# 011235813/discrete_mean_field_game

Measured on AMD Instinct MI355X. Metric: env-steps/sec for batched d-bin population rollouts, higher is better.
Workload: dtype f32 (f64 accumulate); 1 GPU; actor_critic.train(update_every="rollout") of the drop-in class (mfg_ac2.train call surface; device-side start draw every episode, one update per 15-step rollout): d=21 topics, T=15, global batch 65536 = 65536 trajectories per GPU x 1; d=21, T=15, batch_per_gpu=65536, global_batch=65536, rng=philox4x32-10, parallelism=trajectory-sharded x1, 1 all-reduce/update

## Files before the change

### discrete_mean_field_game_amd/csrc/mfg_grad.h

```cpp
#pragma once
#include <hip/hip_runtime.h>
#include <stdint.h>

#include "mfg_core.h"

using namespace mfg;

constexpr int MFG_GRAD_SMALL_MAX_D = 28;
constexpr int GR_OUT_PER_THREAD = 4;
constexpr int GR_OUT_PER_BLOCK = GR_OUT_PER_THREAD * BLOCK;

struct GradArgs {
  const float* pi;
  int64_t stride_b;
  const double* delta;
  const double* g;
  const float* reward;
  int64_t N;
  int T, d, chunk;
  int64_t nsb;
  double* partial;
  int add_reward;
  unsigned* counter;
  double* G;
  int accumulate, apply;
  double lr_c, lr_a;
  double *w, *theta, *reward_acc;
};

__device__ __forceinline__ void grad_partial_body(const GradArgs& a) {
  extern __shared__ __attribute__((aligned(16))) unsigned char smem_raw[];
  const int d = a.d, Q = d * (d + 1) / 2, F = Q + d + 1, FO = F + 3;
  double* dl = reinterpret_cast<double*>(smem_raw);
  float* sp = reinterpret_cast<float*>(dl + 3 * a.chunk);
  const int tid = threadIdx.x;
  int oi[GR_OUT_PER_THREAD], oj[GR_OUT_PER_THREAD], kind[GR_OUT_PER_THREAD];
  double acc[GR_OUT_PER_THREAD];
#pragma unroll
  for (int u = 0; u < GR_OUT_PER_THREAD; ++u) {
    const int k = blockIdx.y * GR_OUT_PER_BLOCK + u * BLOCK + tid;
    acc[u] = 0.0;
    oi[u] = oj[u] = 0;
    if (k < Q) {
      int i = (int)(((2.0 * d + 1.0) - sqrt((2.0 * d + 1.0) * (2.0 * d + 1.0) - 8.0 * (double)k)) * 0.5);
      while (i > 0 && feat_idx(i, i, d) > k) --i;
      while (i + 1 < d && feat_idx(i + 1, i + 1, d) <= k) ++i;
      oi[u] = i;
      oj[u] = i + (k - feat_idx(i, i, d));
      kind[u] = 0;
    } else if (k < Q + d) {
      oi[u] = k - Q;
      kind[u] = 1;
    } else if (k < FO) {
      kind[u] = 2 + (k - (Q + d));
    } else {
      kind[u] = -1;
    }
  }
  for (int64_t n0 = (int64_t)blockIdx.x * a.chunk; n0 < a.N; n0 += a.nsb * a.chunk) {
    const int cn = (int)((a.N - n0) < a.chunk ? (a.N - n0) : a.chunk);
    __syncthreads();
    for (int k = tid; k < cn * d; k += BLOCK) {
      const int q = k / d, c = k - q * d;
      const int64_t n = n0 + q;
      const int64_t b = n / a.T;
      const int s = (int)(n - b * a.T);
      sp[k] = a.pi[b * a.stride_b + (int64_t)s * d + c];
    }
    for (int q = tid; q < cn; q += BLOCK) {
      const double de = a.delta[n0 + q];
      dl[3 * q] = de;
      dl[3 * q + 1] = a.g ? de * a.g[n0 + q] : 0.0;
      dl[3 * q + 2] = a.reward ? (double)a.reward[n0 + q] : 0.0;
    }
    __syncthreads();
#pragma unroll
    for (int u = 0; u < GR_OUT_PER_THREAD; ++u) {
      double s_ = acc[u];
      if (kind[u] == 0) {
        for (int q = 0; q < cn; ++q) s_ = fma(dl[3 * q] * (double)sp[q * d + oi[u]], (double)sp[q * d + oj[u]], s_);
      } else if (kind[u] == 1) {
        for (int q = 0; q < cn; ++q) s_ = fma(dl[3 * q], (double)sp[q * d + oi[u]], s_);
      } else if (kind[u] == 2) {
        for (int q = 0; q < cn; ++q) s_ += dl[3 * q];
      } else if (kind[u] == 3) {
        for (int q = 0; q < cn; ++q) s_ += dl[3 * q + 1];
      } else if (kind[u] == 4) {
        for (int q = 0; q < cn; ++q) s_ += dl[3 * q + 2];
      } else if (kind[u] == 5) {
        s_ += (double)cn;
      }
      acc[u] = s_;
    }
  }
#pragma unroll
  for (int u = 0; u < GR_OUT_PER_THREAD; ++u) {
    const int k = blockIdx.y * GR_OUT_PER_BLOCK + u * BLOCK + tid;
    if (kind[u] >= 0) a.partial[(int64_t)blockIdx.x * FO + k] = acc[u];
  }
}

constexpr int GS_CH = 64;
#ifndef MFG_GS_BPC
#define MFG_GS_BPC 2
#endif

template <int D>
struct GradChunk {
  static constexpr int NL = D ? D : MFG_GRAD_SMALL_MAX_D;
  float pi[NL];
  double de, dg;
  float rr;
};

constexpr int MFG_GRAD_LONG_T = 1 << 22;
__device__ __forceinline__ int grad_boundaries_wide(int sj, int T, float invT) {
  return T >= GS_CH ? (int)(sj >= T) : (int)(((float)sj + 0.5f) * invT);
}
template <int D, bool WIDE>
__device__ __forceinline__ void grad_chunk_load(GradChunk<D>& c, const GradArgs& a, const double* gp, const float* rp, int d,
                                                int64_t n0, int64_t b0, int s0, int lane, float invT, float inv_d) {
  const int last = (int)((a.N - 1 - n0) < (GS_CH - 1) ? (a.N - 1 - n0) : (GS_CH - 1));
  {
    const int64_t n = n0 + (lane < last ? lane : last);
    c.de = a.delta[n];
    c.dg = gp[n];
    c.rr = rp[n];
  }
  if constexpr (!WIDE) {
    const float* cb = a.pi + b0 * a.stride_b + (int64_t)s0 * d;
    const int extra = (int)(a.stride_b - (int64_t)a.T * d);
#pragma unroll
    for (int k = 0; k < GradChunk<D>::NL; ++k) {
      if (!D && k * WAVE >= GS_CH * d) {
        c.pi[k] = 0.0f;
        continue;
      }
      int e = k * WAVE + lane;
      int j = (int)(((float)e + 0.5f) * inv_d);
      if (j > last) { j = last; e = last * d; }
      const int q = (int)(((float)(s0 + j) + 0.5f) * invT);
      c.pi[k] = cb[(unsigned)(e + __mul24(q, extra))];
    }
  } else {
#pragma unroll
    for (int k = 0; k < GradChunk<D>::NL; ++k) {
      if (!D && k * WAVE >= GS_CH * d) {
        c.pi[k] = 0.0f;
        continue;
      }
      const int e = k * WAVE + lane;
      int j = (int)(((float)e + 0.5f) * inv_d);
      int col = e - j * d;
      if (j > last) { j = last; col = 0; }
      const int sj = s0 + j;
      const int q = grad_boundaries_wide(sj, a.T, invT);
      const int64_t off = (b0 + q) * a.stride_b + ((int64_t)(sj - q * a.T) * d + col);
      c.pi[k] = a.pi[off];
    }
  }
}

template <int D, bool WIDE>
__device__ __forceinline__ void grad_mfma_small_body(const GradArgs& a) {
  const int d = D ? D : a.d;
  const int Q = d * (d + 1) / 2, F = Q + d + 1, FO = F + 3;
  constexpr int DMAX = D ? D : MFG_GRAD_SMALL_MAX_D;
  constexpr int PI_FL = GS_CH * DMAX + 16;
  constexpr int W_BYTES = ((PI_FL * 4 + 15) / 16) * 16 + GS_CH * 3 * 8;
  constexpr int RED_BYTES = WAVES * 3 * 4 * WAVE * 8;
  __shared__ __attribute__((aligned(16))) unsigned char smem[(WAVES * W_BYTES > RED_BYTES) ? WAVES * W_BYTES : RED_BYTES];
  const int tid = threadIdx.x, lane = tid & (WAVE - 1), wv = __builtin_amdgcn_readfirstlane(tid / WAVE);
  float* lpi = reinterpret_cast<float*>(smem + (size_t)wv * W_BYTES);
  double* lsc = reinterpret_cast<double*>(smem + (size_t)wv * W_BYTES + ((PI_FL * 4 + 15) / 16) * 16);
  const int li = lane & 15, lk = lane >> 4;
  auto consts = [&](int idx, float& a_d, double& a_1, float& b_1, double& b_g, double& b_r) {
    a_d = idx == d ? 1.0f : 0.0f;
    a_1 = idx == d + 1 ? 1.0 : 0.0;
    b_1 = (idx == d || idx == d + 3) ? 1.0f : 0.0f;
    b_g = idx == d + 1 ? 1.0 : 0.0;
    b_r = idx == d + 2 ? 1.0 : 0.0;
  };
  float ad_lo, b1_lo, ad_hi, b1_hi;
  double a1_lo, a1_hi, bg_lo, br_lo, bg_hi, br_hi;
  consts(li, ad_lo, a1_lo, b1_lo, bg_lo, br_lo);
  consts(16 + li, ad_hi, a1_hi, b1_hi, bg_hi, br_hi);
  const bool pi_lo = li < d, pi_hi = 16 + li < d;
  const int ilo = pi_lo ? li : 0, ihi = pi_hi ? 16 + li : 0;
  const bool has_g = a.g != nullptr, has_r = a.reward != nullptr;
  const double* gp = has_g ? a.g : a.delta;
  const float* rp = has_r ? a.reward : a.pi;
  v4d_t c00 = (v4d_t)(0.0), c01 = (v4d_t)(0.0), c11 = (v4d_t)(0.0);
  const float invT = 1.0f / (float)a.T, inv_d = 1.0f / (float)d;
  const int64_t NC = (a.N + GS_CH - 1) / GS_CH;
  const int64_t W = (int64_t)gridDim.x * WAVES;
  const int64_t gw = (int64_t)blockIdx.x * WAVES + wv;
  GradChunk<D> nx;
  if (gw < NC) grad_chunk_load<D, WIDE>(nx, a, gp, rp, d, gw * GS_CH, (gw * GS_CH) / a.T, (int)((gw * GS_CH) % a.T), lane, invT, inv_d);
  for (int64_t ch = gw; ch < NC; ch += W) {
    const int64_t n0 = ch * GS_CH;
    __builtin_amdgcn_s_waitcnt(0xc07f);
    __builtin_amdgcn_wave_barrier();
#pragma unroll
    for (int k = 0; k < GradChunk<D>::NL; ++k)
      if (D || k * WAVE < GS_CH * d) lpi[k * WAVE + lane] = nx.pi[k];
    {
      const bool ok = n0 + lane < a.N;
      const double rr = (ok && has_r) ? (double)nx.rr : 0.0;
      double de = ok ? nx.de : 0.0;
      if (a.add_reward) {
        de += rr;
        if (ok) const_cast<double*>(a.delta)[n0 + lane] = de;
      }
      lsc[3 * lane] = de;
      lsc[3 * lane + 1] = (ok && has_g) ? nx.dg : 0.0;
      lsc[3 * lane + 2] = rr;
    }
    const int nvalid = (int)((a.N - n0) < GS_CH ? (a.N - n0) : GS_CH);
    if (ch + W < NC) {
      const int64_t n1 = (ch + W) * GS_CH;
      grad_chunk_load<D, WIDE>(nx, a, gp, rp, d, n1, n1 / a.T, (int)(n1 % a.T), lane, invT, inv_d);
    }
    __builtin_amdgcn_s_waitcnt(0xc07f);
    __builtin_amdgcn_wave_barrier();
#pragma unroll 4
    for (int ks = 0; ks < GS_CH / 4; ++ks) {
      const int j = 4 * ks + lk;
      const float plo = lpi[j * d + ilo], phi = lpi[j * d + ihi];
      const double de = lsc[3 * j], dg = lsc[3 * j + 1];
      const double rr = lsc[3 * j + 2];
      const double one = j < nvalid ? 1.0 : 0.0;
      double A_lo, B_lo;
      if constexpr (D >= 16) {
        B_lo = (double)plo;
        A_lo = de * B_lo;
      } else {
        A_lo = fma(de, (double)(pi_lo ? plo : ad_lo), a1_lo * one);
        B_lo = fma(bg_lo, dg, fma(br_lo, rr, (double)(pi_lo ? plo : b1_lo)));
      }
      const double A_hi = fma(de, (double)(pi_hi ? phi : ad_hi), a1_hi * one);
      const double B_hi = fma(bg_hi, dg, fma(br_hi, rr, (double)(pi_hi ? phi : b1_hi)));
      c00 = __builtin_amdgcn_mfma_f64_16x16x4f64(A_lo, B_lo, c00, 0, 0, 0);
      c01 = __builtin_amdgcn_mfma_f64_16x16x4f64(A_lo, B_hi, c01, 0, 0, 0);
      c11 = __builtin_amdgcn_mfma_f64_16x16x4f64(A_hi, B_hi, c11, 0, 0, 0);
    }
  }
  __syncthreads();
  double (*red)[3][4][WAVE] = reinterpret_cast<double (*)[3][4][WAVE]>(smem);
#pragma unroll
  for (int v = 0; v < 4; ++v) {
    red[wv][0][v][lane] = c00[v];
    red[wv][1][v][lane] = c01[v];
    red[wv][2][v][lane] = c11[v];
  }
  __syncthreads();
  double* out = a.partial + (int64_t)blockIdx.x * FO;
  for (int e = tid; e < 3 * 4 * WAVE; e += BLOCK) {
    const int t = e / (4 * WAVE), v = (e / WAVE) & 3, l = e & (WAVE - 1);
    const int gi = (t == 2 ? 16 : 0) + 4 * v + (l >> 4), gj = (t == 0 ? 0 : 16) + (l & 15);
    int k = -1;
    if (gj < d) {
      if (gi <= gj) k = feat_idx(gi, gj, d);
    } else if (gj == d) {
      if (gi <= d) k = Q + gi;
    } else if (gj == d + 1) {
      if (gi == d) k = F;
    } else if (gj == d + 2) {
      if (gi == d + 1) k = F + 1;
    } else if (gj == d + 3) {
      if (gi == d + 1) k = F + 2;
    }
    if (k >= 0) {
      double tsum = red[0][t][v][l];
#pragma unroll
      for (int q = 1; q < WAVES; ++q) tsum += red[q][t][v][l];
      out[k] = tsum;
    }
  }
  if (!a.counter) return;
  __shared__ int s_last;
  __threadfence();
  __syncthreads();
  if (tid == 0) s_last = (atomicAdd(a.counter, 1u) == gridDim.x - 1) ? 1 : 0;
  __syncthreads();
  if (!s_last) return;
  __threadfence();
  double* fin = &red[0][0][0][0];
  const int nrows = (int)gridDim.x;
  for (int k = tid; k < FO; k += BLOCK) {
    double s0 = 0.0, s1 = 0.0, s2 = 0.0, s3 = 0.0;
    const double* col = a.partial + k;
    int r = 0;
    for (; r + 7 < nrows; r += 8) {
      const double v0 = col[(int64_t)r * FO], v1 = col[(int64_t)(r + 1) * FO], v2 = col[(int64_t)(r + 2) * FO],
                   v3 = col[(int64_t)(r + 3) * FO], v4 = col[(int64_t)(r + 4) * FO], v5 = col[(int64_t)(r + 5) * FO],
                   v6 = col[(int64_t)(r + 6) * FO], v7 = col[(int64_t)(r + 7) * FO];
      s0 += v0;
      s1 += v1;
      s2 += v2;
      s3 += v3;
      s0 += v4;
      s1 += v5;
      s2 += v6;
      s3 += v7;
    }
    for (; r < nrows; ++r) s0 += col[(int64_t)r * FO];
    const double tot = (s0 + s1) + (s2 + s3);
    const double gk = a.accumulate ? a.G[k] + tot : tot;
    a.G[k] = gk;
    fin[k] = gk;
  }
  __syncthreads();
  if (a.apply) {
    const double count = fin[F + 2];
    if (count > 0.0) {
      const double inv = 1.0 / count;
      for (int k = tid; k < F; k += BLOCK) a.w[k] = updated_param(a.w[k], a.lr_c, fin[k], inv);
      if (tid == 0) {
        if (a.reward_acc) *a.reward_acc += fin[F + 1] * inv;
        *a.theta = updated_param(*a.theta, a.lr_a, fin[F], inv);
      }
    }
  }
  if (tid == 0) *a.counter = 0u;
}
template <int D, bool WIDE = false>
__global__ __launch_bounds__(BLOCK) void k_grad_mfma_small(GradArgs a) { grad_mfma_small_body<D, WIDE>(a); }

constexpr int GM_KC = 32;
#ifndef MFG_GM_TPW
#define MFG_GM_TPW 8
#endif
constexpr int GM_TPW = MFG_GM_TPW;

template <int NPF>
__device__ __forceinline__ void grad_mfma_body(const GradArgs& a, int tpw) {
  extern __shared__ __attribute__((aligned(16))) unsigned char smem_raw[];
  const int d = a.d, nt = d >> 4, pitch = d + 16;
  const int Q = d * (d + 1) / 2, F = Q + d + 1, FO = F + 3;
  double* dl = reinterpret_cast<double*>(smem_raw);
  double* red = dl + GM_KC;
  float* sp = reinterpret_cast<float*>(red + 4 * BLOCK);
  const int tid = threadIdx.x, lane = tid & (WAVE - 1), wv = tid / WAVE;
  const int ntiles = nt * (nt + 1) / 2;
  const int t0 = ((int)blockIdx.y * WAVES + wv) * tpw;
  int nmine = ntiles - t0;
  nmine = nmine < 0 ? 0 : (nmine > tpw ? tpw : nmine);
  int tr[GM_TPW], tc[GM_TPW];
#pragma unroll
  for (int i = 0; i < GM_TPW; ++i) {
    int t = t0 + i, r = 0;
    if (i < nmine) {
      while (t >= nt - r) {
        t -= nt - r;
        ++r;
      }
    } else {
      t = 0;
    }
    tr[i] = r;
    tc[i] = r + t;
  }
  v4d_t acc[GM_TPW];
#pragma unroll
  for (int i = 0; i < GM_TPW; ++i) acc[i] = (v4d_t)(0.0);
  const bool side = blockIdx.y == 0;
  double lin[4] = {0.0, 0.0, 0.0, 0.0}, s_d = 0.0, s_dg = 0.0, s_r = 0.0, s_n = 0.0;
  const int li = lane & 15, lk = lane >> 4;
  const double invT = 1.0 / (double)a.T;
  const int dq = d >> 2, rpp = BLOCK / (dq > 0 ? dq : 1);
  const int q0 = tid / dq, c4 = tid - q0 * dq;
  float4 pf[NPF > 0 ? NPF : 1];
  double pf_de = 0.0, pf_dg = 0.0, pf_rr = 0.0;
  bool pf_on = false;
#define MFG_GM_FETCH(n0_)                                                                              \
  {                                                                                                    \
    const int cn_ = (int)((a.N - (n0_)) < GM_KC ? (a.N - (n0_)) : GM_KC);                              \
    _Pragma("unroll") for (int u = 0; u < NPF; ++u) {                                                  \
      const int q = q0 + u * rpp;                                                                      \
      pf[u] = make_float4(0.f, 0.f, 0.f, 0.f);                                                         \
      if (q < cn_) {                                                                                   \
        const int64_t n = (n0_) + q;                                                                   \
        const int64_t b = (int64_t)(((double)n + 0.5) * invT);                                         \
        pf[u] = *reinterpret_cast<const float4*>(a.pi + b * a.stride_b + (n - b * a.T) * d + 4 * c4);  \
      }                                                                                                \
    }                                                                                                  \
    pf_de = 0.0; pf_dg = 0.0; pf_rr = 0.0; pf_on = false;                                              \
    if (tid < cn_) {                                                                                   \
      const int64_t n = (n0_) + tid;                                                                   \
      pf_de = a.delta[n];                                                                              \
      pf_rr = a.reward ? (double)a.reward[n] : 0.0;                                                    \
      if (a.g) pf_dg = a.g[n];                                                                         \
      pf_on = true;                                                                                    \
    }                                                                                                  \
  }
  if (NPF > 0 && (int64_t)blockIdx.x * GM_KC < a.N) MFG_GM_FETCH((int64_t)blockIdx.x * GM_KC)
  for (int64_t n0 = (int64_t)blockIdx.x * GM_KC; n0 < a.N; n0 += (int64_t)gridDim.x * GM_KC) {
    const int cn = (int)((a.N - n0) < GM_KC ? (a.N - n0) : GM_KC);
    __syncthreads();
    if (NPF > 0) {
#pragma unroll
      for (int u = 0; u < NPF; ++u) *reinterpret_cast<float4*>(sp + (q0 + u * rpp) * pitch + 4 * c4) = pf[u];
      if (tid < GM_KC) {
        if (side && pf_on) {
          s_d += pf_de;
          if (a.g) s_dg = fma(pf_de, pf_dg, s_dg);
          s_r += pf_rr;
          s_n += 1.0;
        }
        dl[tid] = pf_de;
      }
      __syncthreads();
      const int64_t nn = n0 + (int64_t)gridDim.x * GM_KC;
      if (nn < a.N) MFG_GM_FETCH(nn)
    } else {
    if (a.chunk) {
      for (int q = q0; q < GM_KC; q += rpp) {
        float4 v = make_float4(0.f, 0.f, 0.f, 0.f);
        if (q < cn) {
          const int64_t n = n0 + q;
          const int64_t b = (int64_t)(((double)n + 0.5) * invT);
          v = *reinterpret_cast<const float4*>(a.pi + b * a.stride_b + (n - b * a.T) * d + 4 * c4);
        }
        *reinterpret_cast<float4*>(sp + q * pitch + 4 * c4) = v;
      }
    } else {
      for (int k = tid; k < GM_KC * d; k += BLOCK) {
        const int q = k / d, c = k - q * d;
        float v = 0.0f;
        if (q < cn) {
          const int64_t n = n0 + q;
          const int64_t b = (int64_t)(((double)n + 0.5) * invT);
          v = a.pi[b * a.stride_b + (n - b * a.T) * d + c];
        }
        sp[q * pitch + c] = v;
      }
    }
    if (tid < GM_KC) {
      double de = 0.0;
      if (tid < cn) {
        const int64_t n = n0 + tid;
        de = a.delta[n];
        const double rr = a.reward ? (double)a.reward[n] : 0.0;
        if (side) {
          s_d += de;
          if (a.g) s_dg = fma(de, a.g[n], s_dg);
          s_r += rr;
          s_n += 1.0;
        }
      }
      dl[tid] = de;
    }
    __syncthreads();
    }
#pragma unroll
    for (int ks = 0; ks < GM_KC / 4; ++ks) {
      const int k = ks * 4 + lk;
      const double dk = dl[k];
      const float* row = sp + k * pitch + li;
#pragma unroll
      for (int i = 0; i < GM_TPW; ++i) {
        if (i < nmine) {
          const double av = dk * (double)row[tr[i] << 4];
          const double bv = (double)row[tc[i] << 4];
          acc[i] = __builtin_amdgcn_mfma_f64_16x16x4f64(av, bv, acc[i], 0, 0, 0);
        }
      }
    }
    if (side) {
#pragma unroll
      for (int u = 0; u < 4; ++u) {
        const int c = tid + u * BLOCK;
        if (c < d) {
          double t = lin[u];
          for (int q = 0; q < GM_KC; ++q) t = fma(dl[q], (double)sp[q * pitch + c], t);
          lin[u] = t;
        }
      }
    }
  }
#undef MFG_GM_FETCH
  double* out = a.partial + (int64_t)blockIdx.x * FO;
#pragma unroll
  for (int i = 0; i < GM_TPW; ++i) {
    if (i < nmine) {
#pragma unroll
      for (int v = 0; v < 4; ++v) {
        const int gi = (tr[i] << 4) + 4 * v + lk, gj = (tc[i] << 4) + li;
        if (gi <= gj) out[feat_idx(gi, gj, d)] = acc[i][v];
      }
    }
  }
  if (side) {
#pragma unroll
    for (int u = 0; u < 4; ++u) {
      const int c = tid + u * BLOCK;
      if (c < d) out[Q + c] = lin[u];
    }
    __syncthreads();
    red[tid] = s_d;
    red[BLOCK + tid] = s_dg;
    red[2 * BLOCK + tid] = s_r;
    red[3 * BLOCK + tid] = s_n;
    __syncthreads();
    if (tid < 4) {
      double t = 0.0;
      for (int q = 0; q < GM_KC; ++q) t += red[tid * BLOCK + q];
      out[Q + d + tid] = t;
    }
  }
}
template <int NPF>
__global__ __launch_bounds__(BLOCK) void k_grad_mfma(GradArgs a, int tpw) { grad_mfma_body<NPF>(a, tpw); }

constexpr int RP_SLICES = 64, RP_OUT = 16;
struct ReduceApply {
  double lr_c, lr_a, count;
  double *w, *theta, *reward_acc;
  int on;
};
__device__ __forceinline__ void reduce_partials_body(const double* __restrict__ partial, int64_t nsb, int64_t FO, int accumulate,
                                                     double* __restrict__ G, const ReduceApply& ap) {
  __shared__ double red[RP_SLICES][RP_OUT + 1];
  const int lo = threadIdx.x & (RP_OUT - 1), sl = threadIdx.x / RP_OUT;
  const int64_t k = (int64_t)blockIdx.x * RP_OUT + lo;
  double old_val = 0.0, old_G = 0.0;
  if (sl == 0 && k < FO) {
    const int64_t F = FO - 3;
    if (accumulate) old_G = G[k];
    if (ap.on) {
      if (k < F) old_val = ap.w[k];
      else if (k == F) old_val = *ap.theta;
      else if (k == F + 1 && ap.reward_acc) old_val = *ap.reward_acc;
    }
  }
  double s = 0.0;
  if (k < FO) {
    double s0 = 0.0, s1 = 0.0, s2 = 0.0, s3 = 0.0;
    int64_t p = sl;
    for (; p + 7 * RP_SLICES < nsb; p += 8 * RP_SLICES) {
      const double v0 = partial[p * FO + k], v1 = partial[(p + RP_SLICES) * FO + k], v2 = partial[(p + 2 * RP_SLICES) * FO + k],
                   v3 = partial[(p + 3 * RP_SLICES) * FO + k], v4 = partial[(p + 4 * RP_SLICES) * FO + k],
                   v5 = partial[(p + 5 * RP_SLICES) * FO + k], v6 = partial[(p + 6 * RP_SLICES) * FO + k],
                   v7 = partial[(p + 7 * RP_SLICES) * FO + k];
      s0 += v0;
      s1 += v1;
      s2 += v2;
      s3 += v3;
      s0 += v4;
      s1 += v5;
      s2 += v6;
      s3 += v7;
    }
    double t[7];
#pragma unroll
    for (int u = 0; u < 7; ++u) t[u] = (p + u * RP_SLICES < nsb) ? partial[(p + u * RP_SLICES) * FO + k] : 0.0;
    s0 += t[0];
    s1 += t[1];
    s2 += t[2];
    s3 += t[3];
    s0 += t[4];
    s1 += t[5];
    s2 += t[6];
    s = (s0 + s1) + (s2 + s3);
  }
  red[sl][lo] = s;
  __syncthreads();
  if (sl == 0 && k < FO) {
    double t0 = 0.0, t1 = 0.0, t2 = 0.0, t3 = 0.0;
#pragma unroll
    for (int q = 0; q < RP_SLICES; q += 4) {
      t0 += red[q][lo];
      t1 += red[q + 1][lo];
      t2 += red[q + 2][lo];
      t3 += red[q + 3][lo];
    }
    const double tot = (t0 + t1) + (t2 + t3);
    const double gk = accumulate ? old_G + tot : tot;
    G[k] = gk;
    if (ap.on) {
      const int64_t F = FO - 3;
      const double inv = 1.0 / ap.count;
      if (k < F) ap.w[k] = updated_param(old_val, ap.lr_c, gk, inv);
      else if (k == F) *ap.theta = updated_param(old_val, ap.lr_a, gk, inv);
      else if (k == F + 1 && ap.reward_acc) *ap.reward_acc = old_val + gk * inv;
    }
  }
}
```

### discrete_mean_field_game_amd/csrc/mfg_population.hip

```cpp
#include "mfg_core.h"
#include "mfg_grad.h"
#include "mfg_population.h"
#include "mfg_population_core.h"

namespace mfg {

int launch_core_pop(const CoreArgs& a, const PopArgs& p, bool fast, int num_cus, hipStream_t st) {
  return p.state ? launch_core_pop_ctl(a, p, fast, num_cus, st) : launch_core_pop_forms<false>(a, p, fast, num_cus, st);
}

__global__ void k_draw_start_pop(const float* __restrict__ mat, int64_t num_start, int64_t B, int d, uint32_t step,
                                 uint64_t traj_offset, float* __restrict__ out, PopArgs p) {
  const int k = blockIdx.y;
  draw_start_body(mat, num_start, B, d, p.seed[k], step, traj_offset, nullptr, out + p.s_state * k);
}
__global__ void k_draw_start_pop_ctl(const float* __restrict__ mat, int64_t num_start, int64_t B, int d, uint32_t step,
                                     uint64_t traj_offset, float* __restrict__ out, PopArgs p) {
  const int k = blockIdx.y;
  if (pop_retired(p, k)) return;
  draw_start_body(mat, num_start, B, d, p.seed[k], step, traj_offset, nullptr, out + p.s_state * k);
}

void launch_draw_start_pop(int grid, const float* mat, int64_t num_start, int64_t B, int d, uint32_t step, uint64_t traj_offset,
                           float* out, const PopArgs& p, hipStream_t st) {
  hipLaunchKernelGGL(p.state ? k_draw_start_pop_ctl : k_draw_start_pop, dim3((unsigned)grid, (unsigned)p.K), dim3(256), 0, st, mat,
                     num_start, B, d, step, traj_offset, out, p);
}

__device__ __forceinline__ void pop_rebase_grad(GradArgs& a, const PopArgs& p, int k) {
  a.pi += p.s_gpi * k;
  a.delta += p.s_n * k;
  a.g += p.s_n * k;
  a.reward = pop_at(a.reward, p.s_n, k);
  a.partial = pop_bytes(a.partial, p.s_ws, k);
  a.counter = pop_bytes(a.counter, p.s_ws, k);
  a.G = pop_at(a.G, p.F + 3, k);
  a.w = pop_at(a.w, p.F, k);
  a.theta = pop_at(a.theta, 1, k);
  a.reward_acc = pop_at(a.reward_acc, p.s_acc, k);
  a.lr_c = p.lr_c[k] * p.sc;
  a.lr_a = p.lr_a[k] * p.sa;
}

template <int D>
__global__ __launch_bounds__(BLOCK) void k_grad_mfma_small_pop(GradArgs a, PopArgs p) {
  GradArgs b = a;
  pop_rebase_grad(b, p, blockIdx.y);
  grad_mfma_small_body<D, false>(b);
}
template <int D>
__global__ __launch_bounds__(BLOCK) void k_grad_mfma_small_pop_ctl(GradArgs a, PopArgs p) {
  if (pop_retired(p, blockIdx.y)) return;
  GradArgs b = a;
  pop_rebase_grad(b, p, blockIdx.y);
  grad_mfma_small_body<D, false>(b);
}

__global__ __launch_bounds__(BLOCK) void k_grad_partial_pop(GradArgs a, PopArgs p) {
  GradArgs b = a;
  pop_rebase_grad(b, p, blockIdx.z);
  grad_partial_body(b);
}
__global__ __launch_bounds__(BLOCK) void k_grad_partial_pop_ctl(GradArgs a, PopArgs p) {
  if (pop_retired(p, blockIdx.z)) return;
  GradArgs b = a;
  pop_rebase_grad(b, p, blockIdx.z);
  grad_partial_body(b);
}

template <int NPF>
__global__ __launch_bounds__(BLOCK) void k_grad_mfma_pop(GradArgs a, int tpw, PopArgs p) {
  GradArgs b = a;
  pop_rebase_grad(b, p, blockIdx.z);
  grad_mfma_body<NPF>(b, tpw);
}
template <int NPF>
__global__ __launch_bounds__(BLOCK) void k_grad_mfma_pop_ctl(GradArgs a, int tpw, PopArgs p) {
  if (pop_retired(p, blockIdx.z)) return;
  GradArgs b = a;
  pop_rebase_grad(b, p, blockIdx.z);
  grad_mfma_body<NPF>(b, tpw);
}

#define MFG_REDUCE_PARTIALS_POP()                                                                                        \
  ReduceApply q = ap;                                                                                                    \
  if (q.on) {                                                                                                            \
    q.w = pop_at(ap.w, p.F, k);                                                                                          \
    q.theta = pop_at(ap.theta, 1, k);                                                                                    \
    q.reward_acc = pop_at(ap.reward_acc, p.s_acc, k);                                                                    \
    q.lr_c = p.lr_c[k] * p.sc;                                                                                           \
    q.lr_a = p.lr_a[k] * p.sa;                                                                                           \
  }                                                                                                                      \
                         \
  reduce_partials_body(reinterpret_cast<const double*>(reinterpret_cast<const char*>(partial) + p.s_ws * k), nsb, FO, 0, \
                       G + FO * k, q)
__global__ __launch_bounds__(RP_SLICES* RP_OUT) void k_reduce_partials_pop(const double* __restrict__ partial, int64_t nsb,
                                                                          int64_t FO, double* __restrict__ G, ReduceApply ap,
                                                                          PopArgs p) {
  const int k = blockIdx.y;
  MFG_REDUCE_PARTIALS_POP();
}
__global__ __launch_bounds__(RP_SLICES* RP_OUT) void k_reduce_partials_pop_ctl(const double* __restrict__ partial, int64_t nsb,
                                                                              int64_t FO, double* __restrict__ G, ReduceApply ap,
                                                                              PopArgs p) {
  const int k = blockIdx.y;
  if (pop_retired(p, k)) return;
  MFG_REDUCE_PARTIALS_POP();
}
#undef MFG_REDUCE_PARTIALS_POP

void launch_grad_mfma_small_pop(int D, unsigned blocks, const GradArgs& a, const PopArgs& p, hipStream_t st) {
  const dim3 grid(blocks, (unsigned)p.K);
  auto* k = D == 21   ? (p.state ? k_grad_mfma_small_pop_ctl<21> : k_grad_mfma_small_pop<21>)
            : D == 15 ? (p.state ? k_grad_mfma_small_pop_ctl<15> : k_grad_mfma_small_pop<15>)
                      : (p.state ? k_grad_mfma_small_pop_ctl<0> : k_grad_mfma_small_pop<0>);
  hipLaunchKernelGGL(k, grid, dim3(BLOCK), 0, st, a, p);
}

void launch_grad_partial_pop(unsigned nsb, unsigned nob, size_t lds, const GradArgs& a, const PopArgs& p, hipStream_t st) {
  hipLaunchKernelGGL(p.state ? k_grad_partial_pop_ctl : k_grad_partial_pop, dim3(nsb, nob, (unsigned)p.K), dim3(BLOCK), lds, st, a,
                     p);
}

void launch_grad_mfma_pop(int npf, unsigned nsb, unsigned ny, size_t lds, const GradArgs& a, int tpw, const PopArgs& p,
                          hipStream_t st) {
  const dim3 grid(nsb, ny, (unsigned)p.K);
  auto* k = npf == 2 ? (p.state ? k_grad_mfma_pop_ctl<2> : k_grad_mfma_pop<2>) : (p.state ? k_grad_mfma_pop_ctl<0> : k_grad_mfma_pop<0>);
  hipLaunchKernelGGL(k, grid, dim3(BLOCK), lds, st, a, tpw, p);
}

void launch_reduce_partials_pop(unsigned nob, const double* partial, int64_t nsb, int64_t FO, double* G, const ReduceApply& ap,
                                const PopArgs& p, hipStream_t st) {
  hipLaunchKernelGGL(p.state ? k_reduce_partials_pop_ctl : k_reduce_partials_pop, dim3(nob, (unsigned)p.K),
                     dim3(RP_SLICES * RP_OUT), 0, st, partial, nsb, FO, G, ap, p);
}

__global__ __launch_bounds__(BLOCK) void k_reduce_rows_apply_pop(const double* __restrict__ rows, int nrows, int64_t FO,
                                                                 double* __restrict__ G, double count, double* __restrict__ w,
                                                                 const double* theta_in, double* theta_out,
                                                                 double* __restrict__ reward_acc, double* slots, PopArgs p) {
  const int k = blockIdx.y;
  reduce_rows_apply_body(pop_bytes(rows, p.s_ws, k), nrows, FO, G + FO * k, p.lr_c[k] * p.sc, p.lr_a[k] * p.sa, count,
                         w + p.F * k, pop_bytes(theta_in, p.s_theta_b, k), theta_out + k, pop_at(reward_acc, p.s_acc, k),
                         pop_bytes(slots, p.s_ws, k));
}
__global__ __launch_bounds__(BLOCK) void k_reduce_rows_apply_pop_ctl(const double* __restrict__ rows, int nrows, int64_t FO,
                                                                     double* __restrict__ G, double count,
                                                                     double* __restrict__ w, const double* theta_in,
                                                                     double* theta_out, double* __restrict__ reward_acc,
                                                                     double* slots, PopArgs p) {
  const int k = blockIdx.y;
  if (pop_retired(p, k)) return;
  reduce_rows_apply_body(pop_bytes(rows, p.s_ws, k), nrows, FO, G + FO * k, p.lr_c[k] * p.sc, p.lr_a[k] * p.sa, count,
                         w + p.F * k, pop_bytes(theta_in, p.s_theta_b, k), theta_out + k, pop_at(reward_acc, p.s_acc, k),
                         pop_bytes(slots, p.s_ws, k));
}

void launch_reduce_rows_apply_pop(const double* rows, int nrows, int64_t FO, double* G, double count, double* w,
                                  const double* theta_in, double* theta_out, double* reward_acc, double* slots, const PopArgs& p,
                                  hipStream_t st) {
  hipLaunchKernelGGL(p.state ? k_reduce_rows_apply_pop_ctl : k_reduce_rows_apply_pop,
                     dim3((unsigned)((FO + WAVES - 1) / WAVES), (unsigned)p.K), dim3(BLOCK), 0, st, rows, nrows, FO, G, count, w,
                     theta_in, theta_out, reward_acc, slots, p);
}

__global__ __launch_bounds__(WAVE) void k_pop_retire(mfg_pop_control_t c, const double* __restrict__ theta,
                                                     const double* __restrict__ w, int64_t F, const double* __restrict__ shift,
                                                     int mixed, int after_episode) {
  const int k = blockIdx.x, lane = threadIdx.x;
  if (c.state[k] != 0) return;
  const double th = theta[k];
  bool nonfinite = !isfinite(th);
  for (int64_t j = lane; j < F; j += WAVE) nonfinite |= !isfinite(w[F * k + j]);
  nonfinite = __any(nonfinite);
  const bool range = mixed && !(fabs(th) * (1.0 + fabs(shift[k])) <= SEP_LIMIT);
  if (lane != 0) return;
  const unsigned bits = (mixed ? c.status[k] : 0u) | (range ? (unsigned)MFG_STATUS_MIXED_RANGE : 0u) |
                        (nonfinite ? (unsigned)MFG_STATUS_POP_NONFINITE : 0u);
  if (bits) {
    c.status[k] = bits;
    c.state[k] = 2;
    return;
  }
  if (after_episode) {
    c.episodes_run[k] += 1;
    if (fabs(th - c.theta_prev[k]) < c.stop_criteria[k]) c.state[k] = 1;
  }
  c.theta_prev[k] = th;
}

void launch_pop_retire(const mfg_pop_control_t& c, const double* theta, const double* w, int64_t F, const double* shift, bool mixed,
                       bool after_episode, hipStream_t st) {
  hipLaunchKernelGGL(k_pop_retire, dim3((unsigned)c.K), dim3(WAVE), 0, st, c, theta, w, F, shift, mixed ? 1 : 0,
                     after_episode ? 1 : 0);
}

}
```

Measured before the change: 1.114 billion env-steps/s.

## Software-pipeline LDS reads and MFMA in small grad kernel, precompute chunk geometry

Restructures the inner K loop of the small-d MFMA gradient kernel into groups of four steps. The next group's LDS reads are issued while the current group's operands are built, and sched_barriers separate the MFMA bursts. A fast path for full chunks uses per-lane row indices packed into registers, so the pi gather avoids per-element float division and clamping. Launch bounds now request MFG_GS_BPC blocks per CU. The changes target LDS latency and address arithmetic on the critical path, at the cost of more live registers. Ablation macros are added for experiments but are off by default.

New measurement: 1.115 billion env-steps/s (median of 6 runs). About the same (+0.1%).

```diff
diff --git a/discrete_mean_field_game_amd/csrc/mfg_grad.h b/discrete_mean_field_game_amd/csrc/mfg_grad.h
--- a/discrete_mean_field_game_amd/csrc/mfg_grad.h
+++ b/discrete_mean_field_game_amd/csrc/mfg_grad.h
@@ -105,6 +105,9 @@
 #define MFG_GS_BPC 2
 #endif
 
+constexpr int GS_GK = 4;
+#define MFG_GS_LAUNCH_BOUNDS __launch_bounds__(BLOCK, MFG_GS_BPC)
+
 template <int D>
 struct GradChunk {
   static constexpr int NL = D ? D : MFG_GRAD_SMALL_MAX_D;
@@ -113,14 +116,58 @@
   float rr;
 };
 
+template <int D>
+struct GradGeom {
+  static constexpr int NW = (GradChunk<D>::NL + 3) / 4;
+  unsigned jp[NW];
+};
+template <int D>
+__device__ __forceinline__ void grad_geom_init(GradGeom<D>& gm, int d, int lane, float inv_d) {
+#pragma unroll
+  for (int w = 0; w < GradGeom<D>::NW; ++w) gm.jp[w] = 0u;
+#pragma unroll
+  for (int k = 0; k < GradChunk<D>::NL; ++k) {
+    const int e = k * WAVE + lane;
+    int j = (int)(((float)e + 0.5f) * inv_d);
+    if (!D && k >= d) j = 0;
+    gm.jp[k >> 2] |= (unsigned)j << (8 * (k & 3));
+  }
+}
+
 constexpr int MFG_GRAD_LONG_T = 1 << 22;
 __device__ __forceinline__ int grad_boundaries_wide(int sj, int T, float invT) {
   return T >= GS_CH ? (int)(sj >= T) : (int)(((float)sj + 0.5f) * invT);
 }
 template <int D, bool WIDE>
 __device__ __forceinline__ void grad_chunk_load(GradChunk<D>& c, const GradArgs& a, const double* gp, const float* rp, int d,
-                                                int64_t n0, int64_t b0, int s0, int lane, float invT, float inv_d) {
+                                                int64_t n0, int64_t b0, int s0, int lane, float invT, float inv_d,
+                                                const GradGeom<D>& gm) {
   const int last = (int)((a.N - 1 - n0) < (GS_CH - 1) ? (a.N - 1 - n0) : (GS_CH - 1));
+  if (!WIDE && last == GS_CH - 1) {
+    const int64_t n = n0 + lane;
+    c.de = a.delta[n];
+    c.dg = gp[n];
+    c.rr = rp[n];
+    const float* cb = a.pi + b0 * a.stride_b + (int64_t)s0 * d;
+    const int extra = (int)(a.stride_b - (int64_t)a.T * d);
+    const float s0h = (float)s0 + 0.5f;
+#pragma unroll
+    for (int k = 0; k < GradChunk<D>::NL; ++k) {
+      if (!D && k >= d) {
+        c.pi[k] = 0.0f;
+        continue;
+      }
+      const float jf = (float)((gm.jp[k >> 2] >> (8 * (k & 3))) & 0xffu);
+      const int q = (int)((jf + s0h) * invT);
+#ifdef MFG_GS_ABL_NOADDR
+      c.pi[k] = cb[(unsigned)(k * WAVE + lane)];
+      (void)q, (void)extra;
+#else
+      c.pi[k] = cb[(unsigned)(k * WAVE + lane + __mul24(q, extra))];
+#endif
+    }
+    return;
+  }
   {
     const int64_t n = n0 + (lane < last ? lane : last);
     c.de = a.delta[n];
@@ -195,8 +242,16 @@
   const int64_t NC = (a.N + GS_CH - 1) / GS_CH;
   const int64_t W = (int64_t)gridDim.x * WAVES;
   const int64_t gw = (int64_t)blockIdx.x * WAVES + wv;
+#ifdef MFG_GS_ABL_NOBUILD
+  float abl_f = 1e-3f * (float)lane;
+  double abl_d = 1e-3 * (double)lane;
+  asm volatile("" : "+v"(abl_f), "+v"(abl_d));
+#endif
+  GradGeom<D> gm;
+  if constexpr (!WIDE) grad_geom_init<D>(gm, d, lane, inv_d);
   GradChunk<D> nx;
-  if (gw < NC) grad_chunk_load<D, WIDE>(nx, a, gp, rp, d, gw * GS_CH, (gw * GS_CH) / a.T, (int)((gw * GS_CH) % a.T), lane, invT, inv_d);
+  if (gw < NC)
+    grad_chunk_load<D, WIDE>(nx, a, gp, rp, d, gw * GS_CH, (gw * GS_CH) / a.T, (int)((gw * GS_CH) % a.T), lane, invT, inv_d, gm);
   for (int64_t ch = gw; ch < NC; ch += W) {
     const int64_t n0 = ch * GS_CH;
     __builtin_amdgcn_s_waitcnt(0xc07f);
@@ -217,32 +272,87 @@
       lsc[3 * lane + 2] = rr;
     }
     const int nvalid = (int)((a.N - n0) < GS_CH ? (a.N - n0) : GS_CH);
+#ifndef MFG_GS_ABL_NOLOAD
     if (ch + W < NC) {
       const int64_t n1 = (ch + W) * GS_CH;
-      grad_chunk_load<D, WIDE>(nx, a, gp, rp, d, n1, n1 / a.T, (int)(n1 % a.T), lane, invT, inv_d);
-    }
+      grad_chunk_load<D, WIDE>(nx, a, gp, rp, d, n1, n1 / a.T, (int)(n1 % a.T), lane, invT, inv_d, gm);
+    }
+#endif
     __builtin_amdgcn_s_waitcnt(0xc07f);
     __builtin_amdgcn_wave_barrier();
+    struct Raw {
+      float plo, phi;
+      double de, dg, rr;
+    };
+    struct Opr {
+      double A_lo, B_lo, A_hi, B_hi;
+    };
+    auto k_read = [&](int ks) {
+      const int j = 4 * ks + lk;
+      Raw r;
+#ifdef MFG_GS_ABL_NOBUILD
+      r.plo = r.phi = abl_f;
+      r.de = r.dg = r.rr = abl_d;
+#else
+      r.plo = lpi[j * d + ilo];
+      r.phi = lpi[j * d + ihi];
+      r.de = lsc[3 * j];
+      r.dg = lsc[3 * j + 1];
+      r.rr = lsc[3 * j + 2];
+#endif
+      return r;
+    };
+    auto k_build = [&](const Raw& r, int ks) {
+      Opr o;
+#ifdef MFG_GS_ABL_NOBUILD
+      o.A_lo = o.B_lo = o.A_hi = o.B_hi = r.de;
+#else
+      const int j = 4 * ks + lk;
+      const double one = j < nvalid ? 1.0 : 0.0;
+      if constexpr (D >= 16) {
+        o.B_lo = (double)r.plo;
+        o.A_lo = r.de * o.B_lo;
+      } else {
+        o.A_lo = fma(r.de, (double)(pi_lo ? r.plo : ad_lo), a1_lo * one);
+        o.B_lo = fma(bg_lo, r.dg, fma(br_lo, r.rr, (double)(pi_lo ? r.plo : b1_lo)));
+      }
+      o.A_hi = fma(r.de, (double)(pi_hi ? r.phi : ad_hi), a1_hi * one);
+      o.B_hi = fma(bg_hi, r.dg, fma(br_hi, r.rr, (double)(pi_hi ? r.phi : b1_hi)));
+#endif
+      return o;
+    };
+    auto k_mfma = [&](const Opr& o) {
+#ifdef MFG_GS_ABL_NOMFMA
+      asm volatile("" ::"v"(o.A_lo), "v"(o.B_lo), "v"(o.A_hi), "v"(o.B_hi));
+#else
+      c00 = __builtin_amdgcn_mfma_f64_16x16x4f64(o.A_lo, o.B_lo, c00, 0, 0, 0);
+      c01 = __builtin_amdgcn_mfma_f64_16x16x4f64(o.A_lo, o.B_hi, c01, 0, 0, 0);
+      c11 = __builtin_amdgcn_mfma_f64_16x16x4f64(o.A_hi, o.B_hi, c11, 0, 0, 0);
+#endif
+    };
+    constexpr int NKS = GS_CH / 4;
+    if constexpr (D != 0) {
+      static_assert(NKS % GS_GK == 0, "GS_GK must divide the 16 K steps of a chunk");
+      Raw raw[GS_GK];
+#pragma unroll
+      for (int u = 0; u < GS_GK; ++u) raw[u] = k_read(u);
+#pragma unroll
+      for (int g0 = 0; g0 < NKS; g0 += GS_GK) {
+        Opr op[GS_GK];
+#pragma unroll
+        for (int u = 0; u < GS_GK; ++u) op[u] = k_build(raw[u], g0 + u);
+        if (g0 + GS_GK < NKS) {
+#pragma unroll
+          for (int u = 0; u < GS_GK; ++u) raw[u] = k_read(g0 + GS_GK + u);
+        }
+        __builtin_amdgcn_sched_barrier(0);
+#pragma unroll
+        for (int u = 0; u < GS_GK; ++u) k_mfma(op[u]);
+        __builtin_amdgcn_sched_barrier(0);
+      }
+    } else {
 #pragma unroll 4
-    for (int ks = 0; ks < GS_CH / 4; ++ks) {
-      const int j = 4 * ks + lk;
-      const float plo = lpi[j * d + ilo], phi = lpi[j * d + ihi];
-      const double de = lsc[3 * j], dg = lsc[3 * j + 1];
-      const double rr = lsc[3 * j + 2];
-      const double one = j < nvalid ? 1.0 : 0.0;
-      double A_lo, B_lo;
-      if constexpr (D >= 16) {
-        B_lo = (double)plo;
-        A_lo = de * B_lo;
-      } else {
-        A_lo = fma(de, (double)(pi_lo ? plo : ad_lo), a1_lo * one);
-        B_lo = fma(bg_lo, dg, fma(br_lo, rr, (double)(pi_lo ? plo : b1_lo)));
-      }
-      const double A_hi = fma(de, (double)(pi_hi ? phi : ad_hi), a1_hi * one);
-      const double B_hi = fma(bg_hi, dg, fma(br_hi, rr, (double)(pi_hi ? phi : b1_hi)));
-      c00 = __builtin_amdgcn_mfma_f64_16x16x4f64(A_lo, B_lo, c00, 0, 0, 0);
-      c01 = __builtin_amdgcn_mfma_f64_16x16x4f64(A_lo, B_hi, c01, 0, 0, 0);
-      c11 = __builtin_amdgcn_mfma_f64_16x16x4f64(A_hi, B_hi, c11, 0, 0, 0);
+      for (int ks = 0; ks < NKS; ++ks) k_mfma(k_build(k_read(ks), ks));
     }
   }
   __syncthreads();
@@ -325,7 +435,7 @@
   if (tid == 0) *a.counter = 0u;
 }
 template <int D, bool WIDE = false>
-__global__ __launch_bounds__(BLOCK) void k_grad_mfma_small(GradArgs a) { grad_mfma_small_body<D, WIDE>(a); }
+__global__ MFG_GS_LAUNCH_BOUNDS void k_grad_mfma_small(GradArgs a) { grad_mfma_small_body<D, WIDE>(a); }
 
 constexpr int GM_KC = 32;
 #ifndef MFG_GM_TPW
diff --git a/discrete_mean_field_game_amd/csrc/mfg_population.hip b/discrete_mean_field_game_amd/csrc/mfg_population.hip
--- a/discrete_mean_field_game_amd/csrc/mfg_population.hip
+++ b/discrete_mean_field_game_amd/csrc/mfg_population.hip
@@ -43,13 +43,13 @@
 }
 
 template <int D>
-__global__ __launch_bounds__(BLOCK) void k_grad_mfma_small_pop(GradArgs a, PopArgs p) {
+__global__ MFG_GS_LAUNCH_BOUNDS void k_grad_mfma_small_pop(GradArgs a, PopArgs p) {
   GradArgs b = a;
   pop_rebase_grad(b, p, blockIdx.y);
   grad_mfma_small_body<D, false>(b);
 }
 template <int D>
-__global__ __launch_bounds__(BLOCK) void k_grad_mfma_small_pop_ctl(GradArgs a, PopArgs p) {
+__global__ MFG_GS_LAUNCH_BOUNDS void k_grad_mfma_small_pop_ctl(GradArgs a, PopArgs p) {
   if (pop_retired(p, blockIdx.y)) return;
   GradArgs b = a;
   pop_rebase_grad(b, p, blockIdx.y);
```
